# RobinBruneau/RNb-NeuS2

Measured on AMD Instinct MI355X. Metric: training rays/s + ms/step, normals-only SDF 64x800^2, higher is better.
Workload: dtype f16 storage / f32 accumulate

## Files before the change

rnb-neus2_amd/csrc/rnb_neus2_hip.hip:

```cpp
#include "kernels_net.cuh"
#include "kernels_ray.cuh"
#include "kernels_mesh.cuh"
#include "kernels_render.cuh"
#include "kernels_mesh_sparse.cuh"
#include "kernels_mesh_clean.cuh"
#include "kernels_mesh_simplify.cuh"
#include "../host/mesh.hpp"

#include <hip/hip_ext.h>

#include <algorithm>
#include <atomic>
#include <chrono>
#include <cmath>
#include <cstdio>
#include <cstdlib>
#include <cstring>
#include <limits>
#include <new>
#include <stdexcept>
#include <random>
#include <string>
#include <vector>

// ... 147 lines not shown
	DevBuf<uint32_t> src_slot;
	bool cin_flow = false;
	bool rgb_split() const { return !cfg.apply_no_albedo && !knobs.fwd_bwd_generic; }
	bool wimg_valid = false;
	DevBuf<float> ray_const;
	DevBuf<uint32_t> unfinished;
	uint32_t fwd_k1 = 48;
	bool fwd_k1_fixed = false;
	bool gen_split = false;
	uint32_t gen_k1 = 0, cur_k1 = 0;
	struct Knobs {
		bool march_narrow = false, fwd_bwd_generic = false, loss_wave_per_ray = false;
		uint32_t march_narrow_from = 18432;
		bool dp_order = false;
		bool loss_scan_fused_always = false;
		bool loss_scan_fused = true;
		bool loss_flat = true;
		bool loss_chain_records = true;
		bool scatter_plain = false;
		int march_skip = 1;
		bool march_skip_narrow = false;
		int march_bbox = 1;
		bool dw_sliced = true;
		bool grid_presort = true;
	} knobs;
	DevBuf<RayLoss> ray_loss;
	DevBuf<McTable> mc_table;
	uint32_t render_cap = 0;
	DevBuf<RenderRay> render_rays[2];
	DevBuf<uint32_t> render_keep, render_scan, render_counts;
	DevBuf<float> render_res, render_coords;
	DevBuf<half_t> render_out;
	DevBuf<half_t> fm;
	DevBuf<uint32_t> g12;
	DevBuf<float> srec, var_partial, dw_partial;
	TrainScratch ts;
	uint32_t dw_nwg = 0, dw_chunk = 0;
	uint32_t fwd_grid = 0;
	bool grads_clean = true;

	Pcg32 rng, density_grid_rng, trainer_rng;
	uint32_t density_grid_ema_step = 0;
	uint32_t training_step = 0, valid_level = 0, rays_per_batch = 0;
	uint32_t measured_batch_size = 0, measured_batch_size_before_compaction = 0, n_rays_total = 0;
	uint32_t optimizer_step_count = 0;
	float lr_factor = 1.f;
	uint32_t cur_n_rays = 0, cur_n_rays_total = 0, local_measured_before = 0, cur_step = 0;
	bool grid_updated = false;
	float prep_ms = 0.f;
	std::chrono::steady_clock::time_point step_start;

	hipStream_t s_march = nullptr, s_dw = nullptr, s_adam = nullptr;
	bool tail_pending = false;
	hipEvent_t ev_loss = nullptr, ev_march = nullptr, ev_fb = nullptr, ev_dw = nullptr, ev_adam = nullptr, ev_tail = nullptr, ev_march_rest = nullptr, ev_all = nullptr, ev_sc[3] = {nullptr, nullptr, nullptr};
	struct { bool valid = false, exchanged = false, dp = false, sharded = false, all_final_recorded = false, dw_joined = true; uint64_t split[2] = {0, 0}, split_mid = 0; int order = 0; } sc;
	struct ScatterGroups { uint32_t e_c = 0, l_fine = 0, Ks[RNB_MAX_LEVELS] = {}; uint64_t k_log2 = 0; } sg;
	hipStream_t backward_stream = nullptr;
	hipStream_t step_stream = nullptr;
	uint64_t dp_split = 0, dp_mid = 0;
	uint64_t param_capacity = 0;
	bool dp_order() const { return cfg.world_size > 1 || knobs.dp_order; }
	struct { bool begun = false, early_done = false; AdamArgs args; } opt;
	struct { bool valid = false, loss_cleared = false; uint32_t n_rays = 0, n_rays_total = 0, max_inference = 0, k1 = 0; bool split = false; } pre;
	struct Readback { double sums[3]; uint32_t counters[4]; uint32_t fwd[2]; uint32_t seq, pad; }* host_rb = nullptr;
	uint32_t rb_seq = 0;
	bool loss_polled = true;
	bool poll_loss() const { return overlap() && !dp_order(); }
	void* host_rb_dev = nullptr;
	bool overlap() const { return cfg.overlap != 0 && !prof.on && s_march != nullptr; }

	NetW net(bool inference) const {
		const half_t* p = inference ? params_ema.p : params_fp16.p;
		NetW n;
		n.sdf_w0 = p + off_sdf;
		n.sdf_w1 = n.sdf_w0 + 64 * 32;
		n.rgb_w0 = p + off_rgb;
		n.rgb_w1 = n.rgb_w0 + 64 * 48;
		n.rgb_w2 = n.rgb_w1 + 64 * 64;
		n.grid = reinterpret_cast<const uint32_t*>(p + off_grid);
		n.variance = p + off_var;
		return n;
	}
	GridMeta meta() const { GridMeta g = grid; g.valid_level = valid_level; return g; }
};

static void discard_premarch(rnb_ctx* c);
static bool prep_due(uint32_t step) {
	const uint32_t n_prep_to_skip = std::min(std::max(step / 16u, 1u), 16u);
	return step % n_prep_to_skip == 0;
}
static void join_tail_host(rnb_ctx* c) {
	if (c->tail_pending) { (void)hipEventSynchronize(c->ev_tail); c->tail_pending = false; }
}

static int check_scan_errors(rnb_ctx* c) {
	const bool rays = c->host_coarse[5] != 0, compact = c->host_coarse[6] != 0;
	if (!rays && !compact) return RNB_OK;
	c->host_coarse[5] = 0; c->host_coarse[6] = 0;
	g_err = std::string(rays ? "k_scan_rays_chain" : "k_scan_compact_chain") + ": a tile's sums did not arrive (workgroup not scheduled); the launch reported zero counters";
	return RNB_ERR_DEVICE;
}

namespace {

constexpr size_t LDS_TRAIN = (size_t)(W_TRAIN_END + WAVES_PER_WG * 3 * ACT_TILE_HALFS) * sizeof(half_t);
static_assert(LDS_TRAIN <= 160 * 1024, "training kernel LDS exceeds 160 KiB");

void build_grid_tables(rnb_ctx* c) {
	const rnb_config& cfg = c->cfg;
// ... 552 lines not shown
			DwSlicedArgs q;
			q.n = 0; q.B = B; q.n_slices = n_slices;
			uint32_t wgs = 0;
			auto add_sliced = [&](const half_t* yt, const half_t* xt, float* out, uint32_t n_out, uint32_t n_live, uint32_t n_in, uint32_t ones) {
				q.YT[q.n] = yt; q.XT[q.n] = xt; q.out[q.n] = out; q.n_out[q.n] = n_out; q.n_out_live[q.n] = n_live; q.n_in[q.n] = n_in; q.ones[q.n] = ones;
				q.first_wg[q.n] = wgs; wgs += n_slices * ((n_out * n_in / 4 + 255) / 256); ++q.n;
			};
			if (!a.skip_rgb) {
				add_sliced(T.dh2, T.h1, p_rgb1, 64, 64, 64, 0);
				add_sliced(T.dh1, T.cin, p_rgb0, 64, 64, 32, 0);
				add_sliced(T.dr, T.h2, p_rgb2, 16, 3, 64, 0);
			}
			add_sliced(T.dz, T.sdfin, p_sdf0, 64, 64, 32, 0);
			add_sliced(T.dz1, T.ddin, p_sdf0b, 64, 64, 32, 0);
			add_sliced(T.dso, T.z1, p_sdf1, 16, split ? 16 : 1, 64, 0);
			add_sliced(nullptr, T.front, p_sdf1b, 16, 1, 64, 1);
			for (uint32_t g = q.n; g < 7; ++g) { q.YT[g] = nullptr; q.XT[g] = nullptr; q.out[g] = nullptr; q.n_out[g] = 0; q.n_out_live[g] = 0; q.n_in[g] = 4; q.ones[g] = 0; }
			for (uint32_t g = q.n; g < 8; ++g) q.first_wg[g] = wgs;
			hipLaunchKernelGGL(k_dw_sliced, dim3(wgs), dim3(256), 0, sd, q);
		}
		DwFinishArgs f;
		f.partial[0] = p_rgb2; f.partial[1] = p_rgb1; f.partial[2] = p_rgb0; f.partial[3] = p_sdf1; f.partial[4] = p_sdf0; f.partial[5] = p_sdf0b; f.partial[6] = p_sdf1b;
		f.n_partials = (uint32_t)slab; f.sliced = sliced ? 1u : 0u;
		f.var_partial = c->var_partial.p; f.n_var_partials = fb_grid * WAVES_PER_WG;
		f.grads = c->grads.p; f.grads16 = half ? c->grads16.p : nullptr; f.off_sdf = (uint32_t)c->off_sdf; f.off_rgb = (uint32_t)c->off_rgb; f.off_var = (uint32_t)c->off_var; f.skip_rgb = a.skip_rgb;
		const uint32_t n_fin_blocks = (RNB_N_SDF_MLP_PARAMS + (a.skip_rgb ? 0 : RNB_N_RGB_MLP_PARAMS)) / DWF_PARAMS + 1;
		LAUNCH_EV(k_dw_finish, dim3(n_fin_blocks), dim3(DWF_WG), 0, sd, done, f);
	};

	const uint32_t scatter_cap = (sdf_only && !split) ? 0u : 2u;
	ScatterArgs sa;
	sa.g12 = T.g12; sa.srec = T.srec; sa.B = B; sa.grid_grad = half ? nullptr : c->grads.p + c->off_grid;
	sa.grid_grad16 = half ? reinterpret_cast<uint32_t*>(c->grads16.p + c->off_grid) : nullptr;
	const bool fixed = c->fixed_acc();
	sa.grid_fixed = fixed ? c->grads_fixed.p : nullptr;
	auto narrow = [&](hipStream_t st, hipEvent_t done, uint32_t l0, uint32_t l1) {
		const uint64_t lo = (uint64_t)c->grid.offsets[l0] * 2, hi = (uint64_t)c->grid.offsets[l1] * 2;
		if (hi <= lo) { if (done) (void)hipEventRecord(done, st); return; }
		const uint32_t blocks = (uint32_t)std::min<uint64_t>(2048, ((hi - lo) / 2 + 255) / 256);
		LAUNCH_EV(k_fixed_narrow, dim3(blocks), dim3(256), 0, st, done, c->grads_fixed.p, half ? nullptr : c->grads.p + c->off_grid, half ? c->grads16.p + c->off_grid : nullptr, lo, hi);
	};
	bool sc_first = true;
	auto sc_flags = [&]() -> uint32_t { const bool any = side_streams && !sc_first; sc_first = false; return any ? (uint32_t)hipExtAnyOrderLaunch : 0u; };
	auto launch_a = [&](hipStream_t st, hipEvent_t done, uint32_t l0, uint32_t l1) {
		const uint32_t n_vb = (B * 4 + 255) / 256, cap = scatter_cap ? std::max(1u, (uint32_t)c->n_cus * scatter_cap / std::max(1u, l1 - l0)) : n_vb;
		if (l1 > l0 && fixed) {
			LAUNCH_EVF(k_grid_scatter_quad_fixed, dim3(std::min(n_vb, cap), l1 - l0), dim3(256), 0, st, nullptr, sc_flags(), c->meta(), sa, l0, n_vb);
			narrow(st, done, l0, l1);
		} else if (l1 > l0 && half && c->knobs.scatter_plain) LAUNCH_EVF(k_grid_scatter_quad_h_per_addend, dim3(std::min(n_vb, cap), l1 - l0), dim3(256), 0, st, done, sc_flags(), c->meta(), sa, l0, n_vb);
		else if (l1 > l0 && half) LAUNCH_EVF(k_grid_scatter_quad_h, dim3(std::min(n_vb, cap), l1 - l0), dim3(256), 0, st, done, sc_flags(), c->meta(), sa, l0, n_vb);
		else if (l1 > l0) LAUNCH_EVF(k_grid_scatter_quad, dim3(std::min(n_vb, cap), l1 - l0), dim3(256), 0, st, done, sc_flags(), c->meta(), sa, l0, n_vb);
		else if (done) (void)hipEventRecord(done, st);
	};
	auto launch_b = [&](hipStream_t st, hipEvent_t done) {
		if (l_fine <= e_c) { if (done) (void)hipEventRecord(done, st); return; }
		ScatterRlPlan plan;
		plan.n = l_fine - e_c; plan.k_log2 = sg.k_log2;
		uint32_t wg = 0;
		for (uint32_t q = 0; q < plan.n; ++q) { plan.wg_start[q] = wg; wg += (((B + sg.Ks[e_c + q] - 1) / sg.Ks[e_c + q]) * 4 + 255) / 256; }
		plan.wg_start[plan.n] = wg;
		const uint32_t cap_rl = scatter_cap ? (uint32_t)c->n_cus * scatter_cap : wg;
		const bool staged = c->cur_n_rays != 0 && c->cur_n_rays < c->knobs.march_narrow_from;
		if (fixed) {
			LAUNCH_EVF(k_grid_scatter_quad_rl_fixed, dim3(std::min(wg, cap_rl)), dim3(256), 0, st, nullptr, sc_flags(), c->meta(), sa, e_c, plan);
			narrow(st, done, e_c, l_fine);
		} else if (!staged) {
			if (half) LAUNCH_EVF(k_grid_scatter_quad_rl_direct_h, dim3(std::min(wg, cap_rl)), dim3(256), 0, st, done, sc_flags(), c->meta(), sa, e_c, plan);
			else LAUNCH_EVF(k_grid_scatter_quad_rl_direct_share, dim3(std::min(wg, cap_rl)), dim3(256), 0, st, done, sc_flags(), c->meta(), sa, e_c, plan);
		} else if (half) LAUNCH_EVF(k_grid_scatter_quad_rl_h, dim3(std::min(wg, cap_rl)), dim3(256), LDS_SCATTER_RL, st, done, sc_flags(), c->meta(), sa, e_c, plan);
		else LAUNCH_EVF(k_grid_scatter_quad_rl_share, dim3(std::min(wg, cap_rl)), dim3(256), LDS_SCATTER_RL, st, done, sc_flags(), c->meta(), sa, e_c, plan);
	};
	auto launch_c = [&](hipStream_t st, hipEvent_t done) {
		if (!e_c) { if (done) (void)hipEventRecord(done, st); return; }
		ScatterLdsArgs la; la.a = sa; la.n_levels = e_c;
		const uint32_t wg_cap = 128;
		const uint32_t n_wg = std::max(1u, std::min<uint32_t>(wg_cap, (B + 1023) / 1024));
		la.samples_per_wg = ((B + n_wg - 1) / n_wg + 3) / 4 * 4;
		if (fixed) {
			LAUNCH_EVF(k_grid_scatter_lds_fixed, dim3(n_wg, 2), dim3(512), (size_t)c->grid.offsets[e_c] * 8, st, nullptr, sc_flags(), c->meta(), la);
			narrow(st, done, 0, e_c);
		} else if (half) LAUNCH_EVF(k_grid_scatter_lds_h, dim3(n_wg), dim3(512), (size_t)c->grid.offsets[e_c] * 8, st, done, sc_flags(), c->meta(), la);
		else LAUNCH_EVF(k_grid_scatter_lds, dim3(n_wg), dim3(512), (size_t)c->grid.offsets[e_c] * 8, st, done, sc_flags(), c->meta(), la);
	};

	if (!side_streams) {
		launch_dw(s, nullptr);
		c->prof.mark(s, P_DW);
		launch_c(s, nullptr); c->prof.mark(s, P_SCATTER_LDS);
		launch_b(s, nullptr); c->prof.mark(s, P_SCATTER_RL);
		launch_a(s, nullptr, l_fine, L); c->prof.mark(s, P_SCATTER_QUAD);
		c->prof.units[P_SCATTER_LDS] += B; c->prof.units[P_SCATTER_RL] += B; c->prof.units[P_SCATTER_QUAD] += B;
	} else {
		hipStream_t sd = c->s_dw;
		HIP_TRY(hipStreamWaitEvent(sd, c->ev_fb, 0));
		c->sc.dp = c->dp_order();
		launch_dw(sd, c->ev_dw);
		const uint32_t a_mid = l_fine + (L - l_fine + 1) / 2;
		if (c->sc.dp) launch_c(s, nullptr);
		c->sc.order = (!c->sc.dp && c->cur_n_rays < c->knobs.march_narrow_from && !split) ? 2 : 0;
		if (c->sc.order == 0) {
			launch_b(s, c->ev_sc[0]);
			launch_a(s, c->ev_sc[1], l_fine, a_mid);
			launch_a(s, c->ev_sc[2], a_mid, L);
		} else {
			launch_a(s, c->ev_sc[1], l_fine, L);
			launch_b(s, c->ev_sc[0]);
		}
		c->sc.split_mid = c->off_grid + (uint64_t)c->grid.offsets[a_mid] * 2;
		if (!c->sc.dp) launch_c(s, nullptr);
		if (c->sc.dp || join_dw) HIP_TRY(hipStreamWaitEvent(s, c->ev_dw, 0));
		c->sc.dw_joined = c->sc.dp || join_dw;
		c->sc.valid = true;
		c->sc.split[0] = c->off_grid + (uint64_t)c->grid.offsets[l_fine] * 2;
		c->sc.split[1] = c->off_grid + (uint64_t)c->grid.offsets[e_c] * 2;
	}
	c->prof.units[P_DW] += B;
	c->prof.units[P_SCATTER] += B;
	c->backward_stream = s;
	HIP_TRY(hipGetLastError());
	return RNB_OK;
}

constexpr uint32_t ADAM_LR_TABLE_N = 1u << 16;
static void fill_lr_table(rnb_ctx* c, hipStream_t s) {
	if (c->lr_table_beta1 == c->cfg.beta1 && c->lr_table_beta2 == c->cfg.beta2) return;
	(void)hipDeviceSynchronize();
	hipLaunchKernelGGL(k_adam_lr_table, dim3(ADAM_LR_TABLE_N / 256), dim3(256), 0, s, c->adam_lr_table.p, ADAM_LR_TABLE_N, c->cfg.beta1, c->cfg.beta2);
	(void)hipStreamSynchronize(s);
	c->lr_table_beta1 = c->cfg.beta1; c->lr_table_beta2 = c->cfg.beta2;
}

static int optimizer_begin(rnb_ctx* c) {
	if (c->opt.begun) return RNB_OK;
	const rnb_config& cfg = c->cfg;
	{ const int rc = ensure_opt_records(c); if (rc != RNB_OK) return rc; }
	c->opt_plain_current = false;
	fill_lr_table(c, nullptr);
	const uint32_t step0 = c->optimizer_step_count;
	if (step0 == 0) c->lr_factor = 1.0f;
	if (step0 >= cfg.lr_decay_start && (step0 - cfg.lr_decay_start) % cfg.lr_decay_interval == 0 && step0 <= 10000000u) c->lr_factor *= cfg.lr_decay_base;
	const uint32_t current_step = ++c->optimizer_step_count;
	AdamArgs& a = c->opt.args;
	a.n = c->n_params; a.n_matrix = RNB_N_SDF_MLP_PARAMS + RNB_N_RGB_MLP_PARAMS;
	a.rec = c->opt_rec.p; a.w16 = c->params_fp16.p; a.ema = c->params_ema.p;
	a.grads = c->grads.p; a.grads16 = c->half_acc() ? c->grads16.p : nullptr;
	a.base_lr = cfg.learning_rate * c->lr_factor; a.beta1 = cfg.beta1; a.beta2 = cfg.beta2; a.epsilon = cfg.epsilon; a.l2_reg = cfg.l2_reg;
	a.ema_decay = cfg.ema_decay;
	a.skip_lo = cfg.only_sdf_training ? (uint64_t)c->off_rgb : 0; a.skip_hi = cfg.only_sdf_training ? (uint64_t)c->off_grid : 0;
	a.ema_debias_old = 1 - (float)std::pow(cfg.ema_decay, current_step - 1);
	a.ema_debias_new = 1.0f / (1 - (float)std::pow(cfg.ema_decay, current_step));
	a.lr_table = c->adam_lr_table.p; a.lr_table_n = (uint32_t)c->adam_lr_table.n;
	c->opt.begun = true;
	c->opt.early_done = false;
	return RNB_OK;
}

static void adam_launch(rnb_ctx* c, hipStream_t st, uint64_t lo, uint64_t hi, hipEvent_t done = nullptr) {
	if (hi <= lo) { if (done) (void)hipEventRecord(done, st); return; }
	AdamArgs a = c->opt.args;
	a.begin = lo; a.end = hi;
	const uint32_t blocks = (uint32_t)std::min<uint64_t>(4096, ((hi - lo) / 4 + 255) / 256);
	LAUNCH_EV(k_adam_ema, dim3(blocks), dim3(256), 0, st, done, a);
}
int optimizer_step_early(rnb_ctx* c, hipStream_t st) {
	if (!c->sc.valid || c->opt.early_done) return RNB_OK;
	{ const int rc = optimizer_begin(c); if (rc != RNB_OK) return rc; }
	if (c->sc.dp) adam_launch(c, st, 0, c->sc.split[0], c->ev_adam);
	else adam_launch(c, st, c->sc.split[1], c->sc.split[0], c->ev_adam);
	c->opt.early_done = true;
	HIP_TRY(hipGetLastError());
	return RNB_OK;
}

static void plan_scatter_groups(rnb_ctx* c) {
	rnb_ctx::ScatterGroups& g = c->sg;
	const uint32_t L = c->cfg.n_levels;
	uint32_t l;
	{
		for (l = 0; l < L; ++l) {
			const float run = 590.f / (float)c->grid.resolution[l];
			g.Ks[l] = run >= 5.f ? 16 : run >= 2.5f ? 8 : run >= 1.2f ? 4 : 1;
		}
	}
	if (c->knobs.scatter_plain) {
		for (l = 0; l < L; ++l) g.Ks[l] = 1;
		c->dp_split = c->off_grid; c->dp_mid = c->off_grid + (uint64_t)c->grid.offsets[(L + 1) / 2] * 2;
		return;
	}
	for (l = 0; l < L; ++l) if (l == g.e_c && (size_t)c->grid.offsets[l + 1] * 8 <= 150 * 1024) g.e_c = l + 1;
	g.l_fine = g.e_c;
	for (l = g.e_c; l < L && g.Ks[l] > 1 && l - g.e_c < 16; ++l) {
		g.k_log2 |= (uint64_t)ilog2(g.Ks[l]) << (4 * (l - g.e_c));
		g.l_fine = l + 1;
	}
	c->dp_split = c->off_grid + (uint64_t)c->grid.offsets[g.l_fine] * 2;
	c->dp_mid = c->off_grid + (uint64_t)c->grid.offsets[g.l_fine + (L - g.l_fine + 1) / 2] * 2;
}

static int optimizer_finish(rnb_ctx* c, hipStream_t s, bool images_done = false) {
	c->opt.begun = false;
	c->opt.early_done = false;
	c->sc.valid = false;
	if (!images_done) hipLaunchKernelGGL(k_prepare_weight_images, dim3(WIMG_WGS, 4), dim3(WG), 0, s, c->net(false), c->wimg_fwd.p, c->wimg_fbs.p, c->wimg_train.p, c->wimg_rgb.p, c->half_acc() ? 1 : 0);
	c->wimg_valid = true;
	c->prof.mark(s, P_ADAM);
	c->prof.units[P_ADAM] += (double)c->n_params;
	HIP_TRY(hipGetLastError());
	c->grads_clean = true;
	return RNB_OK;
}

static void shard_layout(const rnb_ctx* c, rnb_shard_part parts[RNB_MAX_SHARD_PARTS], uint32_t* n_parts) {
	const uint64_t W = std::max(1u, c->cfg.world_size), r = c->cfg.rank, q = 4 * W;
	uint32_t n = 0;
	const uint64_t m0 = c->dp_split / q * q, m1 = std::max(m0, c->dp_mid / q * q);
	if (m0) { parts[n].lo = 0; parts[n].hi = m0; ++n; }
	if (m1 > m0 && m1 < c->param_capacity) { parts[n].lo = m0; parts[n].hi = m1; ++n; }
	parts[n].lo = (m1 > m0 && m1 < c->param_capacity) ? m1 : m0; parts[n].hi = c->param_capacity; ++n;
	for (uint32_t k = 0; k < n; ++k) {
		const uint64_t chunk = (parts[k].hi - parts[k].lo) / W;
		parts[k].own_lo = parts[k].lo + r * chunk;
		parts[k].own_hi = parts[k].own_lo + chunk;
	}
	*n_parts = n;
}

int optimizer_step(rnb_ctx* c, hipStream_t s) {
	{ const int rc = optimizer_begin(c); if (rc != RNB_OK) return rc; }
	c->prof.mark(s, P_NONE);
	const bool chunked = !c->opt.early_done && c->overlap() && !c->sc.dp && c->sc.valid && !c->sc.exchanged;
	if (!c->sc.dw_joined && !chunked) {
		HIP_TRY(hipStreamWaitEvent(s, c->ev_dw, 0));
		c->sc.dw_joined = true;
	}
	bool images_done = false;
	if (c->opt.early_done) {
		if (!c->sc.dp) adam_launch(c, s, 0, c->sc.split[1]);
		adam_launch(c, s, c->sc.split[0], c->n_params);
		HIP_TRY(hipStreamWaitEvent(s, c->ev_adam, 0));
	} else if (chunked) {
		hipStream_t sa = c->s_adam;
		if (c->sc.order == 0) {
			HIP_TRY(hipStreamWaitEvent(sa, c->ev_sc[0], 0));
			adam_launch(c, sa, c->sc.split[1], c->sc.split[0]);
			HIP_TRY(hipStreamWaitEvent(sa, c->ev_sc[1], 0));
			adam_launch(c, sa, c->sc.split[0], c->sc.split_mid);
			HIP_TRY(hipStreamWaitEvent(sa, c->ev_sc[2], 0));
			adam_launch(c, sa, c->sc.split_mid, c->off_var, c->ev_adam);
		} else {
			HIP_TRY(hipStreamWaitEvent(sa, c->ev_sc[1], 0));
			adam_launch(c, sa, c->sc.split[0], c->off_var);
			HIP_TRY(hipStreamWaitEvent(sa, c->ev_sc[0], 0));
			adam_launch(c, sa, c->sc.split[1], c->sc.split[0], c->ev_adam);
		}
		if (c->sc.dw_joined) {
			adam_launch(c, s, 0, c->sc.split[1]);
			adam_launch(c, s, c->off_var, c->n_params);
		} else {
			hipStream_t sd = c->s_dw;
			adam_launch(c, sd, 0, c->off_grid);
			adam_launch(c, sd, c->off_var, c->n_params);
			LAUNCH_EV(k_prepare_weight_images, dim3(WIMG_WGS, 4), dim3(WG), 0, sd, c->ev_tail, c->net(false), c->wimg_fwd.p, c->wimg_fbs.p, c->wimg_train.p, c->wimg_rgb.p, c->half_acc() ? 1 : 0);
			images_done = true;
			adam_launch(c, s, c->off_grid, c->sc.split[1]);
			if (!c->pre.valid && !prep_due(c->cur_step + 1)) c->tail_pending = true;
			else HIP_TRY(hipStreamWaitEvent(s, c->ev_tail, 0));
			c->sc.dw_joined = true;
		}
		HIP_TRY(hipStreamWaitEvent(s, c->ev_adam, 0));
	} else {
		adam_launch(c, s, 0, c->n_params);
	}
	return optimizer_finish(c, s, images_done);
}

int optimizer_step_shard(rnb_ctx* c, uint32_t part, hipStream_t st) {
	rnb_shard_part parts[RNB_MAX_SHARD_PARTS];
	uint32_t n = 0;
	shard_layout(c, parts, &n);
	if (part >= n) return fail(RNB_ERR_INVALID, "rnb_train_step_apply_shard: no such block");
	const rnb_shard_part& p = parts[part];
	{ const int rc = optimizer_begin(c); if (rc != RNB_OK) return rc; }
	if (!c->sc.dw_joined) HIP_TRY(hipStreamWaitEvent(st, c->ev_dw, 0));
	if (p.own_lo > p.lo) HIP_TRY(hipMemsetAsync(c->grad_ptr(p.lo), 0, (p.own_lo - p.lo) * c->grad_elem(), st));
	if (p.hi > p.own_hi) HIP_TRY(hipMemsetAsync(c->grad_ptr(p.own_hi), 0, (p.hi - p.own_hi) * c->grad_elem(), st));
	adam_launch(c, st, std::min<uint64_t>(p.own_lo, c->n_params), std::min<uint64_t>(p.own_hi, c->n_params));
	HIP_TRY(hipGetLastError());
	return RNB_OK;
}

hipStream_t as_stream(void* s) { return reinterpret_cast<hipStream_t>(s); }

static int update_config_common(rnb_config& dst, const rnb_config* cfg) {
	if (cfg->abi_version != RNB_ABI_VERSION) return fail(RNB_ERR_INVALID, "abi_version mismatch");
	if (cfg->n_levels != dst.n_levels || cfg->log2_hashmap_size != dst.log2_hashmap_size || cfg->base_resolution != dst.base_resolution ||
	    cfg->per_level_scale != dst.per_level_scale || cfg->target_batch_size != dst.target_batch_size || cfg->max_rays_per_batch != dst.max_rays_per_batch ||
	    cfg->aabb_scale != dst.aabb_scale || cfg->seed != dst.seed || cfg->world_size != dst.world_size || cfg->rank != dst.rank || cfg->accumulate != dst.accumulate || cfg->deterministic != dst.deterministic)
		return fail(RNB_ERR_INVALID, "rnb_update_config: geometry fields differ from the context's");
	dst = *cfg;
	return RNB_OK;
}


}

extern "C" {
#define RNB_GUARD                                                                                                   \
	catch (const std::bad_alloc&) { return fail(RNB_ERR_NOMEM, "out of host memory (std::bad_alloc)"); }                \
	catch (const std::exception& e_) { return fail(RNB_ERR_INVALID, std::string("exception: ") + e_.what()); }          \
	catch (...) { return fail(RNB_ERR_INVALID, "unknown exception"); }

const char* rnb_last_error(void) { return g_err.c_str(); }
uint32_t rnb_abi_version(void) { return RNB_ABI_VERSION; }

int rnb_default_config(rnb_config* cfg) try {
	if (!cfg) return fail(RNB_ERR_INVALID, "cfg is null");
	std::memset(cfg, 0, sizeof(*cfg));
	cfg->abi_version = RNB_ABI_VERSION;
	cfg->n_levels = 14; cfg->log2_hashmap_size = 19; cfg->base_resolution = 16;
	cfg->per_level_scale = std::exp(std::log(2048.0f * 1.0f / 16.0f) / (14 - 1));
	cfg->valid_level_scale = 0.02f; cfg->base_valid_level_scale = 0.2f; cfg->base_training_step = 100;
	cfg->sdf_bias = -0.1f;
	cfg->target_batch_size = 1u << 18; cfg->initial_rays_per_batch = 1u << 12; cfg->max_rays_per_batch = 1u << 18;
	cfg->aabb_scale = 1; cfg->seed = 1337;
	cfg->mask_loss_weight = 1.0f; cfg->ek_loss_weight = 0.01f;
	cfg->apply_L2 = 1; cfg->apply_rgbplus = 1; cfg->apply_no_albedo = 0; cfg->apply_light_opti = 0;
	cfg->apply_supernormal = 0; cfg->apply_relu = 0; cfg->apply_bce = 0; cfg->snap_to_pixel_centers = 1;
	cfg->learning_rate = 1e-3f; cfg->beta1 = 0.9f; cfg->beta2 = 0.99f; cfg->epsilon = 1e-15f; cfg->l2_reg = 1e-6f;
	cfg->ema_decay = 0.95f; cfg->lr_decay_start = 20000; cfg->lr_decay_interval = 10000; cfg->lr_decay_base = 0.33f;
	cfg->density_grid_decay = 0.95f;
	cfg->world_size = 1; cfg->rank = 0;
	cfg->overlap = 1;
	return RNB_OK;
} RNB_GUARD

int rnb_destroy(rnb_ctx* c) try {
	if (!c) return RNB_OK;
	if (c->march_stats.p) {
		unsigned long long h[8] = {0, 0, 0, 0, 0, 0, 0, 0};
		(void)hipDeviceSynchronize();
		if (hipMemcpy(h, c->march_stats.p, sizeof(h), hipMemcpyDeviceToHost) == hipSuccess && h[0])
			fprintf(stderr, "k_march_count_skip: %llu wavefronts, %.2f loop iterations each; %llu rays: %.3f skipped at least once, %.3f ended early, %.5f start-overs per ray, %.3f rounds per ray looking for a re-entry cell\n",
			        h[0], (double)h[1] / h[0], h[2], (double)h[3] / h[2], (double)h[6] / h[2], (double)h[4] / h[2], (double)h[5] / h[2]);
		c->march_stats.free();
	}
	c->opt_rec.free(); c->params_fp32.free(); c->grads.free(); c->grads16.free(); c->grads_fixed.free(); c->adam_m.free(); c->adam_v.free(); c->params_fp16.free(); c->params_ema.free(); c->adam_steps.free(); c->adam_lr_table.free();
	c->density_grid.free(); c->density_grid_tmp.free(); c->density_grid_tmp_alt.free(); c->density_mean.free(); c->mean_partial.free(); c->loss_sums.free(); c->bitfield.free(); c->coarse_bits.free(); c->coarse_count.free();
	c->grid_sample_pos.free(); c->grid_sample_idx.free(); c->views.free(); c->pixels.free();
	c->gs_sorted_pos.free(); c->gs_sorted_idx.free(); c->gs_stage_pos.free(); c->gs_stage_idx.free(); c->gs_hist.free(); c->gs_range.free(); c->gs_eval_pos.free(); c->gs_eval_idx.free();
	c->ray_indices.free(); c->numsteps.free(); c->counters.free(); c->rays.free(); c->coords.free(); c->coords_compacted.free();
	c->loss.free(); c->mlp_out.free(); c->chain_rec.free(); c->ray_grad.free(); c->ray_of.free(); c->slot_of.free(); c->wg_partial.free(); c->dloss_dout.free();
	c->wimg_fwd.free(); c->wimg_fbs.free(); c->wimg_train.free(); c->wimg_rgb.free(); c->cin_eval.free(); c->dcin.free(); c->rgb_out_scratch.free(); c->src_slot.free(); c->ray_const.free(); c->ray_base1.free(); c->scan_words.free(); c->idx1.free(); c->idx2.free(); c->fwd_counts.free(); c->unfinished.free();
	c->ray_setup.free(); c->ray_t.free(); c->ray_dunnorm.free(); c->ray_steps.free(); c->ray_base.free(); c->ray_slot.free(); c->ncomp.free(); c->cbase.free(); c->scan_tiles.free(); c->loss_partial.free(); c->ray_loss.free();
	c->render_rays[0].free(); c->render_rays[1].free(); c->render_keep.free(); c->render_scan.free(); c->render_counts.free(); c->render_res.free(); c->render_coords.free(); c->render_out.free();
	c->mc_table.free(); c->fm.free(); c->g12.free(); c->srec.free(); c->var_partial.free(); c->dw_partial.free();
	c->prof.destroy();
	if (c->s_march) { (void)hipStreamSynchronize(c->s_march); (void)hipStreamDestroy(c->s_march); }
	for (hipStream_t st : {c->s_dw, c->s_adam}) if (st) { (void)hipStreamSynchronize(st); (void)hipStreamDestroy(st); }
	for (hipEvent_t e : {c->ev_loss, c->ev_march, c->ev_fb, c->ev_dw, c->ev_adam, c->ev_tail, c->ev_march_rest, c->ev_all, c->ev_grid, c->ev_gs, c->ev_sc[0], c->ev_sc[1], c->ev_sc[2]}) if (e) (void)hipEventDestroy(e);
	if (c->host_rb) (void)hipHostFree(c->host_rb);
	if (c->host_coarse) (void)hipHostFree(c->host_coarse);
	delete c;
	return RNB_OK;
} RNB_GUARD

int rnb_create(const rnb_config* cfg, rnb_ctx** out) try {
	if (!cfg || !out) return fail(RNB_ERR_INVALID, "null argument");
	if (cfg->abi_version != RNB_ABI_VERSION) return fail(RNB_ERR_INVALID, "abi_version mismatch");
	if (cfg->n_levels == 0 || cfg->n_levels > 14) return fail(RNB_ERR_INVALID, "n_levels must be in [1,14]");
	if (cfg->base_resolution < 2) return fail(RNB_ERR_INVALID, "base_resolution must be >= 2");
	if (cfg->aabb_scale == 0 || (cfg->aabb_scale & (cfg->aabb_scale - 1)) != 0 || cfg->aabb_scale > 128) return fail(RNB_ERR_INVALID, "aabb_scale must be a power of two <= 128");
	if (cfg->target_batch_size == 0 || cfg->target_batch_size % 128 != 0) return fail(RNB_ERR_INVALID, "target_batch_size must be a positive multiple of 128");
	if (cfg->max_rays_per_batch == 0 || cfg->max_rays_per_batch > (1u << 18)) return fail(RNB_ERR_INVALID, "max_rays_per_batch must be in [1, 2^18]");
	if (cfg->world_size == 0 || cfg->rank >= cfg->world_size) return fail(RNB_ERR_INVALID, "bad rank/world_size");
	if (cfg->accumulate > RNB_ACCUM_HALF) return fail(RNB_ERR_INVALID, "accumulate must be RNB_ACCUM_FP32 or RNB_ACCUM_HALF");
	if (cfg->deterministic > 1) return fail(RNB_ERR_INVALID, "deterministic must be 0 or 1");
	if (cfg->accumulate == RNB_ACCUM_HALF && getenv("RNB_FWD_BWD_GENERIC")) return fail(RNB_ERR_INVALID, "RNB_FWD_BWD_GENERIC (the generic training kernel of rounds 1-3) has no half-accumulate form");
	int dev = 0;
	HIP_TRY(hipGetDevice(&dev));
	hipDeviceProp_t prop;
	HIP_TRY(hipGetDeviceProperties(&prop, dev));
	if (std::string(prop.gcnArchName).find("gfx950") == std::string::npos) return fail(RNB_ERR_DEVICE, std::string("librnb_neus2_hip targets gfx950 (MI355X); found ") + prop.gcnArchName);
	rnb_ctx* c = new rnb_ctx();
#define HIP_TRY_C(expr)                                                                                                  \
	do {                                                                                                                 \
		hipError_t e_ = (expr);                                                                                          \
		if (e_ != hipSuccess) { rnb_destroy(c); return fail(RNB_ERR_DEVICE, std::string(#expr) + ": " + hipGetErrorString(e_)); } \
	} while (0)
	c->cfg = *cfg;
	if (const char* e = getenv("RNB_DETERMINISTIC")) c->cfg.deterministic = atoi(e) != 0 ? 1u : 0u;
	c->n_cus = prop.multiProcessorCount;
	build_grid_tables(c);
	c->off_sdf = 0;
	c->off_rgb = RNB_N_SDF_MLP_PARAMS;
	c->off_grid = c->off_rgb + RNB_N_RGB_MLP_PARAMS;
	c->off_var = c->off_grid + c->n_grid_params;
	c->n_params = c->off_var + RNB_N_VARIANCE_PARAMS;
	c->aabb.mn = 0.5f - 0.5f * std::min(1u << (N_CASCADES - 1), cfg->aabb_scale);
	c->aabb.mx = 0.5f + 0.5f * std::min(1u << (N_CASCADES - 1), cfg->aabb_scale);
	c->aabb.max_cascade = 0;
	while ((1u << c->aabb.max_cascade) < cfg->aabb_scale) ++c->aabb.max_cascade;
	c->aabb.cone_angle = cfg->aabb_scale <= 1 ? 0.0f : (1.0f / 256.0f);
	const uint32_t B = cfg->target_batch_size, maxr = cfg->max_rays_per_batch;
	const uint32_t n_grid = GRID_CELLS * (c->aabb.max_cascade + 1);
#define ALLOC(buf, count)                                                                                              \
	do {                                                                                                               \
		if ((buf).alloc(count) != hipSuccess) { rnb_destroy(c); return fail(RNB_ERR_NOMEM, "hipMalloc failed for " #buf); } \
	} while (0)
	{
		const uint64_t q = 4ull * std::max(1u, cfg->world_size);
		c->param_capacity = (c->n_params + q - 1) / q * q;
	}
// ... 61 lines not shown
	if (rc != RNB_OK) { rnb_destroy(c); return rc; }
	HIP_TRY_C(hipFuncSetAttribute(reinterpret_cast<const void*>(k_forward_chained_emul_pipe<4>), hipFuncAttributeMaxDynamicSharedMemorySize, (int)LDS_FWD2));
	HIP_TRY_C(hipFuncSetAttribute(reinterpret_cast<const void*>(k_forward_chained_pipe<4>), hipFuncAttributeMaxDynamicSharedMemorySize, (int)LDS_FWD2));
	HIP_TRY_C(hipFuncSetAttribute(reinterpret_cast<const void*>(k_fwd_bwd), hipFuncAttributeMaxDynamicSharedMemorySize, (int)LDS_TRAIN));
	HIP_TRY_C(hipFuncSetAttribute(reinterpret_cast<const void*>(k_fwd_bwd_sdf), hipFuncAttributeMaxDynamicSharedMemorySize, (int)LDS_FBS));
	HIP_TRY_C(hipFuncSetAttribute(reinterpret_cast<const void*>(k_fwd_bwd_sdf_full), hipFuncAttributeMaxDynamicSharedMemorySize, (int)LDS_FBS_FULL));
	HIP_TRY_C(hipFuncSetAttribute(reinterpret_cast<const void*>(k_rgb_fwd_bwd), hipFuncAttributeMaxDynamicSharedMemorySize, (int)LDS_RGB));
	HIP_TRY_C(hipFuncSetAttribute(reinterpret_cast<const void*>(k_fwd_bwd_sdf_h), hipFuncAttributeMaxDynamicSharedMemorySize, (int)LDS_FBS));
	HIP_TRY_C(hipFuncSetAttribute(reinterpret_cast<const void*>(k_fwd_bwd_sdf_hs), hipFuncAttributeMaxDynamicSharedMemorySize, (int)LDS_FBS));
	HIP_TRY_C(hipFuncSetAttribute(reinterpret_cast<const void*>(k_fwd_bwd_sdf_full_hs), hipFuncAttributeMaxDynamicSharedMemorySize, (int)LDS_FBS_FULL));
	HIP_TRY_C(hipFuncSetAttribute(reinterpret_cast<const void*>(k_rgb_fwd_bwd_hs), hipFuncAttributeMaxDynamicSharedMemorySize, (int)LDS_RGB));
	HIP_TRY_C(hipFuncSetAttribute(reinterpret_cast<const void*>(k_fwd_bwd_sdf_full_h), hipFuncAttributeMaxDynamicSharedMemorySize, (int)LDS_FBS_FULL));
	HIP_TRY_C(hipFuncSetAttribute(reinterpret_cast<const void*>(k_rgb_fwd_bwd_h), hipFuncAttributeMaxDynamicSharedMemorySize, (int)LDS_RGB));
	HIP_TRY_C(hipFuncSetAttribute(reinterpret_cast<const void*>(k_grid_scatter_lds_h), hipFuncAttributeMaxDynamicSharedMemorySize, 150 * 1024));
	{
		const int march_lds_max = (int)((2 * COARSE_WORDS + 2 * COARSE_MAX_BLOCKS) * sizeof(uint32_t));
		HIP_TRY_C(hipFuncSetAttribute(reinterpret_cast<const void*>(k_march_count<true>), hipFuncAttributeMaxDynamicSharedMemorySize, march_lds_max));
		HIP_TRY_C(hipFuncSetAttribute(reinterpret_cast<const void*>(k_march_count_wide<16, true>), hipFuncAttributeMaxDynamicSharedMemorySize, march_lds_max));
		HIP_TRY_C(hipFuncSetAttribute(reinterpret_cast<const void*>(k_march_count_wide<64, true, 256>), hipFuncAttributeMaxDynamicSharedMemorySize, march_lds_max));
		HIP_TRY_C(hipFuncSetAttribute(reinterpret_cast<const void*>(k_march_count_skip<1024>), hipFuncAttributeMaxDynamicSharedMemorySize, march_lds_max + (int)(COARSE_WORDS * sizeof(uint32_t))));
		HIP_TRY_C(hipFuncSetAttribute(reinterpret_cast<const void*>(k_march_count_skip_narrow), hipFuncAttributeMaxDynamicSharedMemorySize, march_lds_max + (int)(COARSE_WORDS * sizeof(uint32_t))));
		HIP_TRY_C(hipFuncSetAttribute(reinterpret_cast<const void*>(k_march_count_bbox), hipFuncAttributeMaxDynamicSharedMemorySize, march_lds_max));
	}
HIP_TRY_C(hipFuncSetAttribute(reinterpret_cast<const void*>(k_grid_scatter_lds), hipFuncAttributeMaxDynamicSharedMemorySize, 150 * 1024));
	HIP_TRY_C(hipFuncSetAttribute(reinterpret_cast<const void*>(k_grid_scatter_lds_fixed), hipFuncAttributeMaxDynamicSharedMemorySize, 150 * 1024));
	c->rng = Pcg32{cfg->seed};
	c->density_grid_rng = Pcg32{c->rng.next_uint()};
	(void)c->rng.next_uint();
	c->rays_per_batch = std::min(cfg->initial_rays_per_batch, cfg->max_rays_per_batch);
	c->training_step = 0;
	c->valid_level = compute_valid_level(c->cfg, 0);
	build_light_dirs(c);
	if (const char* e = getenv("RNB_FWD_K1")) { c->fwd_k1 = (uint32_t)atoi(e); c->fwd_k1_fixed = true; }
	{
		rnb_ctx::Knobs& k = c->knobs;
		k.march_narrow = getenv("RNB_MARCH_NARROW") != nullptr; k.fwd_bwd_generic = getenv("RNB_FWD_BWD_GENERIC") != nullptr;
		k.loss_wave_per_ray = getenv("RNB_LOSS_WAVE_PER_RAY") != nullptr;
		k.dp_order = getenv("RNB_DP_FORCE_COLLECTIVES") != nullptr;
		if (const char* e = getenv("RNB_MARCH_NARROW_FROM")) k.march_narrow_from = (uint32_t)atoi(e);
		if (const char* e = getenv("RNB_GRID_PRESORT")) k.grid_presort = atoi(e) != 0;
		if (const char* e = getenv("RNB_LOSS_SCAN_FUSED")) { k.loss_scan_fused = atoi(e) != 0; k.loss_scan_fused_always = atoi(e) == 2; }
		if (const char* e = getenv("RNB_LOSS_FLAT")) k.loss_flat = atoi(e) != 0;
		if (const char* e = getenv("RNB_LOSS_CHAIN_RECORDS")) k.loss_chain_records = atoi(e) != 0;
		if (const char* e = getenv("RNB_SCATTER_PLAIN")) k.scatter_plain = atoi(e) != 0;
		if (const char* e = getenv("RNB_DW_SLICED")) k.dw_sliced = atoi(e) != 0;
		if (const char* e = getenv("RNB_MARCH_SKIP")) k.march_skip = std::max(0, std::min(2, atoi(e)));
		if (const char* e = getenv("RNB_MARCH_SKIP_NARROW")) k.march_skip_narrow = atoi(e) != 0;
		if (const char* e = getenv("RNB_MARCH_BBOX")) k.march_bbox = std::max(0, std::min(2, atoi(e)));
	}
	plan_scatter_groups(c);
	for (hipStream_t* st : {&c->s_march, &c->s_dw, &c->s_adam}) HIP_TRY_C(hipStreamCreateWithFlags(st, hipStreamNonBlocking));
	HIP_TRY_C(hipEventCreateWithFlags(&c->ev_loss, hipEventDisableTiming));
	const unsigned dev_flags = hipEventDisableTiming | (unsigned)hipEventDisableSystemFence;
	for (hipEvent_t* e : {&c->ev_march, &c->ev_fb, &c->ev_dw, &c->ev_adam, &c->ev_tail, &c->ev_march_rest, &c->ev_all, &c->ev_grid, &c->ev_gs, &c->ev_sc[0], &c->ev_sc[1], &c->ev_sc[2]}) HIP_TRY_C(hipEventCreateWithFlags(e, dev_flags));
	HIP_TRY_C(hipHostMalloc(reinterpret_cast<void**>(&c->host_rb), sizeof(*c->host_rb), hipHostMallocMapped));
	std::memset(c->host_rb, 0, sizeof(*c->host_rb));
	HIP_TRY_C(hipHostGetDevicePointer(&c->host_rb_dev, c->host_rb, 0));
	HIP_TRY_C(hipHostMalloc(reinterpret_cast<void**>(&c->host_coarse), 64, hipHostMallocMapped));
	std::memset(c->host_coarse, 0, 64);
	*c->host_coarse = 0xffffffffu;
	HIP_TRY_C(hipMemset(c->scan_words.p, 0, c->scan_words.bytes()));
	HIP_TRY_C(hipHostGetDevicePointer(reinterpret_cast<void**>(&c->host_coarse_dev), c->host_coarse, 0));
	*out = c;
	return RNB_OK;
#undef HIP_TRY_C
} RNB_GUARD

int rnb_update_config(rnb_ctx* c, const rnb_config* cfg) try {
	if (!c || !cfg) return fail(RNB_ERR_INVALID, "null argument");
	discard_premarch(c);
	int rc = update_config_common(c->cfg, cfg);
	if (rc != RNB_OK) return rc;
	build_light_dirs(c);
	return RNB_OK;
} RNB_GUARD

uint64_t rnb_n_params(const rnb_ctx* c) { return c ? c->n_params : 0; }

int rnb_param_layout(const rnb_ctx* c, uint64_t offsets[5]) try {
	if (!c || !offsets) return fail(RNB_ERR_INVALID, "null argument");
	offsets[0] = c->off_sdf; offsets[1] = c->off_rgb; offsets[2] = c->off_grid; offsets[3] = c->off_var; offsets[4] = c->n_params;
	return RNB_OK;
} RNB_GUARD

int rnb_grid_tables(const rnb_ctx* c, uint32_t* offsets, uint32_t* resolution, float* scale) try {
	if (!c) return fail(RNB_ERR_INVALID, "null ctx");
	for (uint32_t i = 0; i <= c->cfg.n_levels; ++i) if (offsets) offsets[i] = c->grid.offsets[i];
	for (uint32_t i = 0; i < c->cfg.n_levels; ++i) { if (resolution) resolution[i] = c->grid.resolution[i]; if (scale) scale[i] = c->grid.scale[i]; }
	return RNB_OK;
} RNB_GUARD

int rnb_init_params(rnb_ctx* c, const float* sdf_w) try {
	if (!c || !sdf_w) return fail(RNB_ERR_INVALID, "null argument");
	discard_premarch(c);
	HIP_TRY(hipDeviceSynchronize());
	std::seed_seq seq{c->cfg.seed};
	std::vector<uint32_t> seeds(2);
	seq.generate(std::begin(seeds), std::end(seeds));
	Pcg32 rnd{seeds.front()};
	std::vector<float> mlp(RNB_N_SDF_MLP_PARAMS + RNB_N_RGB_MLP_PARAMS, 0.f);
	auto xavier = [&](float* dst, int rows, int cols) {
		float scale = 1.f;
		scale *= std::sqrt(6.0f / (float)(cols + rows));
		for (int i = 0; i < rows * cols; ++i) dst[i] = (float)(rnd.next_float() * 2.0f * scale - scale);
	};
	xavier(mlp.data(), 64, 32);
	xavier(mlp.data() + 64 * 32, 16, 64);
// ... 732 lines not shown
	} else if (c->sc.valid && c->sc.split[1] < c->sc.split[0]) {
		ranges[0][0] = c->sc.split[1]; ranges[0][1] = c->sc.split[0];
		ranges[1][0] = 0;              ranges[1][1] = c->sc.split[1];
		ranges[2][0] = c->sc.split[0]; ranges[2][1] = c->n_params;
		*n_parts = 3;
	} else {
		ranges[0][0] = 0; ranges[0][1] = c->n_params; *n_parts = 1;
	}
	return RNB_OK;
} RNB_GUARD

int rnb_train_step_apply_early(rnb_ctx* c, void* stream) try {
	if (!c) return fail(RNB_ERR_INVALID, "null ctx");
	return optimizer_step_early(c, as_stream(stream));
} RNB_GUARD

int rnb_shard_layout(rnb_ctx* c, rnb_shard_part parts[RNB_MAX_SHARD_PARTS], uint32_t* n_parts, uint64_t* capacity) try {
	if (!c || !parts || !n_parts || !capacity) return fail(RNB_ERR_INVALID, "null argument");
	c->sc.exchanged = true;
	c->sc.sharded = true;
	shard_layout(c, parts, n_parts);
	*capacity = c->param_capacity;
	return RNB_OK;
} RNB_GUARD

int rnb_train_step_apply_shard(rnb_ctx* c, uint32_t part, void* stream) try {
	if (!c) return fail(RNB_ERR_INVALID, "null ctx");
	return optimizer_step_shard(c, part, as_stream(stream));
} RNB_GUARD

int rnb_train_step_apply_done(rnb_ctx* c, void* stream) try {
	if (!c) return fail(RNB_ERR_INVALID, "null ctx");
	if (!c->opt.begun) return fail(RNB_ERR_INVALID, "rnb_train_step_apply_done without rnb_train_step_apply_shard");
	int rc = optimizer_finish(c, as_stream(stream));
	if (rc != RNB_OK) return rc;
	++c->training_step;
	return RNB_OK;
} RNB_GUARD

int rnb_gradient_part_wait(rnb_ctx* c, uint32_t part, void* stream) try {
	if (!c) return fail(RNB_ERR_INVALID, "null ctx");
	const bool early = part == 0 && c->sc.valid && (c->sc.dp || !c->sc.sharded);
	bool mid = false;
	if (part == 1 && c->sc.valid && c->sc.dp) {
		if (c->sc.sharded) { rnb_shard_part parts[RNB_MAX_SHARD_PARTS]; uint32_t n = 0; shard_layout(c, parts, &n); mid = n == 3; }
		else mid = c->sc.split_mid > c->sc.split[0] && c->sc.split_mid < c->off_var;
	}
	if (!c->sc.dw_joined) HIP_TRY(hipStreamWaitEvent(as_stream(stream), c->ev_dw, 0));
	if (!early && !mid && !c->sc.all_final_recorded) {
		HIP_TRY(hipEventRecord(c->ev_all, c->backward_stream));
		c->sc.all_final_recorded = true;
	}
	HIP_TRY(hipStreamWaitEvent(as_stream(stream), early ? c->ev_sc[0] : mid ? c->ev_sc[1] : c->ev_all, 0));
	if (early && c->sc.dp) HIP_TRY(hipStreamWaitEvent(as_stream(stream), c->ev_dw, 0));
	return RNB_OK;
} RNB_GUARD

uint32_t rnb_render_abi_version(void) { return RNB_RENDER_ABI_VERSION; }

int rnb_render_default_options(rnb_render_options* opt) try {
	if (!opt) return fail(RNB_ERR_INVALID, "opt is null");
	std::memset(opt, 0, sizeof(*opt));
	opt->abi_version = RNB_RENDER_ABI_VERSION;
	opt->min_transmittance = 0.01f;
	opt->near_distance = 0.2f;
	opt->use_inference_params = 1;
	opt->use_occupancy = 1;
	opt->max_rays_in_flight = 0;
	return RNB_OK;
} RNB_GUARD

int rnb_render(rnb_ctx* c, void* stream, const rnb_view* view, const rnb_render_options* opt, float* out, rnb_render_stats* stats) try {
	if (!c || !view || !opt) return fail(RNB_ERR_INVALID, "rnb_render: null argument");
	if (opt->abi_version != RNB_RENDER_ABI_VERSION) return fail(RNB_ERR_INVALID, "rnb_render: options abi_version mismatch (expected RNB_RENDER_ABI_VERSION)");
	if (!out) return fail(RNB_ERR_INVALID, "rnb_render: out_dev is null");
	if (view->width == 0 || view->height == 0) return fail(RNB_ERR_INVALID, "rnb_render: empty view");
	const uint64_t n_pix = (uint64_t)view->width * view->height;
	if (n_pix > (1ull << 31)) return fail(RNB_ERR_INVALID, "rnb_render: more than 2^31 pixels");
	if (!(opt->min_transmittance >= 0.f && opt->min_transmittance < 1.f)) return fail(RNB_ERR_INVALID, "rnb_render: min_transmittance must be in [0, 1)");
	if (!(opt->near_distance >= 0.f) || !std::isfinite(opt->near_distance)) return fail(RNB_ERR_INVALID, "rnb_render: near_distance must be finite and >= 0");
	if (!(view->focal_length[0] > 0.f && view->focal_length[1] > 0.f)) return fail(RNB_ERR_INVALID, "rnb_render: focal lengths must be positive");
	const auto t_begin = std::chrono::steady_clock::now();
	hipStream_t s = as_stream(stream);
	join_tail_host(c);

	uint32_t R = opt->max_rays_in_flight ? opt->max_rays_in_flight : (1u << 19);
	R = std::max<uint32_t>(64u, R / 64u * 64u);
	R = (uint32_t)std::min<uint64_t>(R, (n_pix + 63) / 64 * 64);
	if (R > c->render_cap) {
		c->render_rays[0].free(); c->render_rays[1].free(); c->render_keep.free(); c->render_scan.free(); c->render_res.free(); c->render_coords.free(); c->render_out.free();
		c->render_cap = 0;
		if (c->render_rays[0].alloc(R) != hipSuccess || c->render_rays[1].alloc(R) != hipSuccess || c->render_keep.alloc(R) != hipSuccess ||
		    c->render_scan.alloc(scan_scratch_elems(R)) != hipSuccess || c->render_res.alloc((size_t)R * RENDER_RES_FLOATS) != hipSuccess ||
		    c->render_coords.alloc((size_t)R * RENDER_MAX_N * 7) != hipSuccess || c->render_out.alloc((size_t)R * RENDER_MAX_N * 16) != hipSuccess) {
			c->render_rays[0].free(); c->render_rays[1].free(); c->render_keep.free(); c->render_scan.free(); c->render_res.free(); c->render_coords.free(); c->render_out.free();
			return fail(RNB_ERR_NOMEM, "rnb_render: hipMalloc failed for the render workspace (lower max_rays_in_flight)");
		}
		c->render_cap = R;
	}
	if (!c->render_counts.p && c->render_counts.alloc(4) != hipSuccess) return fail(RNB_ERR_NOMEM, "rnb_render: hipMalloc failed for the counters");
	uint32_t* n_eval = c->render_counts.p;
	uint32_t* n_hit = c->render_counts.p + 1;
	unsigned long long* n_samples = reinterpret_cast<unsigned long long*>(c->render_counts.p + 2);
	HIP_TRY(hipMemsetAsync(c->render_counts.p, 0, 16, s));

	RenderArgs a;
// ... 427 lines not shown
```

Baseline: 51.99 million.

## Split row-level grid scatter into two launches so Adam overlaps earlier

The row-level scatter for the middle grid levels is split at a balance point into two kernel launches, each signalling its own event. The chunked Adam stream can then start updating the first half of those parameters while the second half is still being scattered. The aim is to hide more of the optimizer cost behind the backward scatter. In exchange it adds a kernel launch, an event and cross-stream waits, and the two smaller launches may each fill the device less well.

New measurement: 51.44 million. -1.1%, worse.

```diff
diff --git a/rnb-neus2_amd/csrc/rnb_neus2_hip.hip b/rnb-neus2_amd/csrc/rnb_neus2_hip.hip
--- a/rnb-neus2_amd/csrc/rnb_neus2_hip.hip
+++ b/rnb-neus2_amd/csrc/rnb_neus2_hip.hip
@@ -223,9 +223,9 @@
 
 	hipStream_t s_march = nullptr, s_dw = nullptr, s_adam = nullptr;
 	bool tail_pending = false;
-	hipEvent_t ev_loss = nullptr, ev_march = nullptr, ev_fb = nullptr, ev_dw = nullptr, ev_adam = nullptr, ev_tail = nullptr, ev_march_rest = nullptr, ev_all = nullptr, ev_sc[3] = {nullptr, nullptr, nullptr};
-	struct { bool valid = false, exchanged = false, dp = false, sharded = false, all_final_recorded = false, dw_joined = true; uint64_t split[2] = {0, 0}, split_mid = 0; int order = 0; } sc;
-	struct ScatterGroups { uint32_t e_c = 0, l_fine = 0, Ks[RNB_MAX_LEVELS] = {}; uint64_t k_log2 = 0; } sg;
+	hipEvent_t ev_loss = nullptr, ev_march = nullptr, ev_fb = nullptr, ev_dw = nullptr, ev_adam = nullptr, ev_tail = nullptr, ev_march_rest = nullptr, ev_all = nullptr, ev_sc[4] = {nullptr, nullptr, nullptr, nullptr};
+	struct { bool valid = false, exchanged = false, dp = false, sharded = false, all_final_recorded = false, dw_joined = true; uint64_t split[2] = {0, 0}, split_mid = 0, b_first[2] = {0, 0}; int order = 0; } sc;
+	struct ScatterGroups { uint32_t e_c = 0, l_fine = 0, b_mid = 0, Ks[RNB_MAX_LEVELS] = {}; uint64_t k_log2 = 0; } sg;
 	hipStream_t backward_stream = nullptr;
 	hipStream_t step_stream = nullptr;
 	uint64_t dp_split = 0, dp_mid = 0;
@@ -884,23 +884,23 @@
 		else if (l1 > l0) LAUNCH_EVF(k_grid_scatter_quad, dim3(std::min(n_vb, cap), l1 - l0), dim3(256), 0, st, done, sc_flags(), c->meta(), sa, l0, n_vb);
 		else if (done) (void)hipEventRecord(done, st);
 	};
-	auto launch_b = [&](hipStream_t st, hipEvent_t done) {
-		if (l_fine <= e_c) { if (done) (void)hipEventRecord(done, st); return; }
+	auto launch_b = [&](hipStream_t st, hipEvent_t done, uint32_t l0, uint32_t l1) {
+		if (l1 <= l0) { if (done) (void)hipEventRecord(done, st); return; }
 		ScatterRlPlan plan;
-		plan.n = l_fine - e_c; plan.k_log2 = sg.k_log2;
+		plan.n = l1 - l0; plan.k_log2 = sg.k_log2 >> (4 * (l0 - e_c));
 		uint32_t wg = 0;
-		for (uint32_t q = 0; q < plan.n; ++q) { plan.wg_start[q] = wg; wg += (((B + sg.Ks[e_c + q] - 1) / sg.Ks[e_c + q]) * 4 + 255) / 256; }
+		for (uint32_t q = 0; q < plan.n; ++q) { plan.wg_start[q] = wg; wg += (((B + sg.Ks[l0 + q] - 1) / sg.Ks[l0 + q]) * 4 + 255) / 256; }
 		plan.wg_start[plan.n] = wg;
 		const uint32_t cap_rl = scatter_cap ? (uint32_t)c->n_cus * scatter_cap : wg;
 		const bool staged = c->cur_n_rays != 0 && c->cur_n_rays < c->knobs.march_narrow_from;
 		if (fixed) {
-			LAUNCH_EVF(k_grid_scatter_quad_rl_fixed, dim3(std::min(wg, cap_rl)), dim3(256), 0, st, nullptr, sc_flags(), c->meta(), sa, e_c, plan);
-			narrow(st, done, e_c, l_fine);
+			LAUNCH_EVF(k_grid_scatter_quad_rl_fixed, dim3(std::min(wg, cap_rl)), dim3(256), 0, st, nullptr, sc_flags(), c->meta(), sa, l0, plan);
+			narrow(st, done, l0, l1);
 		} else if (!staged) {
-			if (half) LAUNCH_EVF(k_grid_scatter_quad_rl_direct_h, dim3(std::min(wg, cap_rl)), dim3(256), 0, st, done, sc_flags(), c->meta(), sa, e_c, plan);
-			else LAUNCH_EVF(k_grid_scatter_quad_rl_direct_share, dim3(std::min(wg, cap_rl)), dim3(256), 0, st, done, sc_flags(), c->meta(), sa, e_c, plan);
-		} else if (half) LAUNCH_EVF(k_grid_scatter_quad_rl_h, dim3(std::min(wg, cap_rl)), dim3(256), LDS_SCATTER_RL, st, done, sc_flags(), c->meta(), sa, e_c, plan);
-		else LAUNCH_EVF(k_grid_scatter_quad_rl_share, dim3(std::min(wg, cap_rl)), dim3(256), LDS_SCATTER_RL, st, done, sc_flags(), c->meta(), sa, e_c, plan);
+			if (half) LAUNCH_EVF(k_grid_scatter_quad_rl_direct_h, dim3(std::min(wg, cap_rl)), dim3(256), 0, st, done, sc_flags(), c->meta(), sa, l0, plan);
+			else LAUNCH_EVF(k_grid_scatter_quad_rl_direct_share, dim3(std::min(wg, cap_rl)), dim3(256), 0, st, done, sc_flags(), c->meta(), sa, l0, plan);
+		} else if (half) LAUNCH_EVF(k_grid_scatter_quad_rl_h, dim3(std::min(wg, cap_rl)), dim3(256), LDS_SCATTER_RL, st, done, sc_flags(), c->meta(), sa, l0, plan);
+		else LAUNCH_EVF(k_grid_scatter_quad_rl_share, dim3(std::min(wg, cap_rl)), dim3(256), LDS_SCATTER_RL, st, done, sc_flags(), c->meta(), sa, l0, plan);
 	};
 	auto launch_c = [&](hipStream_t st, hipEvent_t done) {
 		if (!e_c) { if (done) (void)hipEventRecord(done, st); return; }
@@ -919,7 +919,7 @@
 		launch_dw(s, nullptr);
 		c->prof.mark(s, P_DW);
 		launch_c(s, nullptr); c->prof.mark(s, P_SCATTER_LDS);
-		launch_b(s, nullptr); c->prof.mark(s, P_SCATTER_RL);
+		launch_b(s, nullptr, e_c, l_fine); c->prof.mark(s, P_SCATTER_RL);
 		launch_a(s, nullptr, l_fine, L); c->prof.mark(s, P_SCATTER_QUAD);
 		c->prof.units[P_SCATTER_LDS] += B; c->prof.units[P_SCATTER_RL] += B; c->prof.units[P_SCATTER_QUAD] += B;
 	} else {
@@ -930,14 +930,20 @@
 		const uint32_t a_mid = l_fine + (L - l_fine + 1) / 2;
 		if (c->sc.dp) launch_c(s, nullptr);
 		c->sc.order = (!c->sc.dp && c->cur_n_rays < c->knobs.march_narrow_from && !split) ? 2 : 0;
+		const uint32_t b_mid = c->sc.dp ? e_c : sg.b_mid;
+		auto launch_b2 = [&]() {
+			if (b_mid > e_c) launch_b(s, c->ev_sc[3], e_c, b_mid);
+			launch_b(s, c->ev_sc[0], b_mid, l_fine);
+		};
 		if (c->sc.order == 0) {
-			launch_b(s, c->ev_sc[0]);
+			launch_b2();
 			launch_a(s, c->ev_sc[1], l_fine, a_mid);
 			launch_a(s, c->ev_sc[2], a_mid, L);
 		} else {
 			launch_a(s, c->ev_sc[1], l_fine, L);
-			launch_b(s, c->ev_sc[0]);
+			launch_b2();
 		}
+		c->sc.b_first[0] = c->off_grid + (uint64_t)c->grid.offsets[e_c] * 2; c->sc.b_first[1] = c->off_grid + (uint64_t)c->grid.offsets[b_mid] * 2;
 		c->sc.split_mid = c->off_grid + (uint64_t)c->grid.offsets[a_mid] * 2;
 		if (!c->sc.dp) launch_c(s, nullptr);
 		if (c->sc.dp || join_dw) HIP_TRY(hipStreamWaitEvent(s, c->ev_dw, 0));
@@ -1025,6 +1031,9 @@
 		g.k_log2 |= (uint64_t)ilog2(g.Ks[l]) << (4 * (l - g.e_c));
 		g.l_fine = l + 1;
 	}
+	g.b_mid = g.e_c;
+	for (l = g.l_fine; l > g.e_c; --l) if (c->grid.offsets[g.l_fine] - c->grid.offsets[l] <= c->grid.offsets[l] - c->grid.offsets[g.e_c]) g.b_mid = l;
+	if (g.b_mid == g.l_fine) g.b_mid = g.e_c;
 	c->dp_split = c->off_grid + (uint64_t)c->grid.offsets[g.l_fine] * 2;
 	c->dp_mid = c->off_grid + (uint64_t)c->grid.offsets[g.l_fine + (L - g.l_fine + 1) / 2] * 2;
 }
@@ -1072,9 +1081,14 @@
 		HIP_TRY(hipStreamWaitEvent(s, c->ev_adam, 0));
 	} else if (chunked) {
 		hipStream_t sa = c->s_adam;
+		const bool b_two = c->sc.b_first[1] > c->sc.b_first[0];
 		if (c->sc.order == 0) {
+			if (b_two) {
+				HIP_TRY(hipStreamWaitEvent(sa, c->ev_sc[3], 0));
+				adam_launch(c, sa, c->sc.b_first[0], c->sc.b_first[1]);
+			}
 			HIP_TRY(hipStreamWaitEvent(sa, c->ev_sc[0], 0));
-			adam_launch(c, sa, c->sc.split[1], c->sc.split[0]);
+			adam_launch(c, sa, c->sc.b_first[1], c->sc.split[0]);
 			HIP_TRY(hipStreamWaitEvent(sa, c->ev_sc[1], 0));
 			adam_launch(c, sa, c->sc.split[0], c->sc.split_mid);
 			HIP_TRY(hipStreamWaitEvent(sa, c->ev_sc[2], 0));
@@ -1082,8 +1096,12 @@
 		} else {
 			HIP_TRY(hipStreamWaitEvent(sa, c->ev_sc[1], 0));
 			adam_launch(c, sa, c->sc.split[0], c->off_var);
+			if (b_two) {
+				HIP_TRY(hipStreamWaitEvent(sa, c->ev_sc[3], 0));
+				adam_launch(c, sa, c->sc.b_first[0], c->sc.b_first[1]);
+			}
 			HIP_TRY(hipStreamWaitEvent(sa, c->ev_sc[0], 0));
-			adam_launch(c, sa, c->sc.split[1], c->sc.split[0], c->ev_adam);
+			adam_launch(c, sa, c->sc.b_first[1], c->sc.split[0], c->ev_adam);
 		}
 		if (c->sc.dw_joined) {
 			adam_launch(c, s, 0, c->sc.split[1]);
@@ -1189,7 +1207,7 @@
 	c->prof.destroy();
 	if (c->s_march) { (void)hipStreamSynchronize(c->s_march); (void)hipStreamDestroy(c->s_march); }
 	for (hipStream_t st : {c->s_dw, c->s_adam}) if (st) { (void)hipStreamSynchronize(st); (void)hipStreamDestroy(st); }
-	for (hipEvent_t e : {c->ev_loss, c->ev_march, c->ev_fb, c->ev_dw, c->ev_adam, c->ev_tail, c->ev_march_rest, c->ev_all, c->ev_grid, c->ev_gs, c->ev_sc[0], c->ev_sc[1], c->ev_sc[2]}) if (e) (void)hipEventDestroy(e);
+	for (hipEvent_t e : {c->ev_loss, c->ev_march, c->ev_fb, c->ev_dw, c->ev_adam, c->ev_tail, c->ev_march_rest, c->ev_all, c->ev_grid, c->ev_gs, c->ev_sc[0], c->ev_sc[1], c->ev_sc[2], c->ev_sc[3]}) if (e) (void)hipEventDestroy(e);
 	if (c->host_rb) (void)hipHostFree(c->host_rb);
 	if (c->host_coarse) (void)hipHostFree(c->host_coarse);
 	delete c;
@@ -1357,7 +1375,7 @@
 	for (hipStream_t* st : {&c->s_march, &c->s_dw, &c->s_adam}) HIP_TRY_C(hipStreamCreateWithFlags(st, hipStreamNonBlocking));
 	HIP_TRY_C(hipEventCreateWithFlags(&c->ev_loss, hipEventDisableTiming));
 	const unsigned dev_flags = hipEventDisableTiming | (unsigned)hipEventDisableSystemFence;
-	for (hipEvent_t* e : {&c->ev_march, &c->ev_fb, &c->ev_dw, &c->ev_adam, &c->ev_tail, &c->ev_march_rest, &c->ev_all, &c->ev_grid, &c->ev_gs, &c->ev_sc[0], &c->ev_sc[1], &c->ev_sc[2]}) HIP_TRY_C(hipEventCreateWithFlags(e, dev_flags));
+	for (hipEvent_t* e : {&c->ev_march, &c->ev_fb, &c->ev_dw, &c->ev_adam, &c->ev_tail, &c->ev_march_rest, &c->ev_all, &c->ev_grid, &c->ev_gs, &c->ev_sc[0], &c->ev_sc[1], &c->ev_sc[2], &c->ev_sc[3]}) HIP_TRY_C(hipEventCreateWithFlags(e, dev_flags));
 	HIP_TRY_C(hipHostMalloc(reinterpret_cast<void**>(&c->host_rb), sizeof(*c->host_rb), hipHostMallocMapped));
 	std::memset(c->host_rb, 0, sizeof(*c->host_rb));
 	HIP_TRY_C(hipHostGetDevicePointer(&c->host_rb_dev, c->host_rb, 0));
@@ -2196,6 +2214,7 @@
 		c->sc.all_final_recorded = true;
 	}
 	HIP_TRY(hipStreamWaitEvent(as_stream(stream), early ? c->ev_sc[0] : mid ? c->ev_sc[1] : c->ev_all, 0));
+	if (early && c->sc.b_first[1] > c->sc.b_first[0]) HIP_TRY(hipStreamWaitEvent(as_stream(stream), c->ev_sc[3], 0));
 	if (early && c->sc.dp) HIP_TRY(hipStreamWaitEvent(as_stream(stream), c->ev_dw, 0));
 	return RNB_OK;
 } RNB_GUARD
```
